# LPD-EPFL-ML/X-MAP

Measured on AMD Instinct MI355X. Metric: item_sim_pairs_per_s, higher is better.
Workload: dtype f64

## Files before the change

x-map_amd/csrc/tri_pairs.hip:

```cpp
#include <type_traits>

#include "tri.h"

namespace xmap {

constexpr uint32_t T_EMPTY = 0xFFFFFFFFu;

struct TriArgs {
    const long long *iptr;
    const RaterRec *rc;
    const int2 *ub;
    const double *u_avg; const double *nrm;
    int cap;
    const int *Q; const uint8_t *small; const int *uq_item; const int *uq_q; long long unit_lo, unit_hi;
    const int *hid; const int *hlist; const int *CH; const int *uc_item; const int *uc_c;
    const long long *uc_ptr; const int *C;
    double *hp_hi; double *hp_lo; int *hp_cnt; int *hp_mut;
    long long shard_cap;
    unsigned long long *shard_cur;
    unsigned long long *shard_occ;
    int *coo_i; int *coo_j; double *coo_sim; int *coo_mutu; int *coo_nij;
    double *coo_aux;
    int *rowcnt;
    int *mircnt;
    unsigned long long *counters;
    int heavy_mod, heavy_rem;
    int raw;
};

template <int METHOD>
__device__ __forceinline__ bool finish_pair(const TriArgs &A, int i, int j, int n, int m, double dot, double &simv) {
    const double np = A.nrm[i] * A.nrm[j];
    const double cs = (np != 0.0) ? 1.0 * dot / np : 0.0;
    const int mn = n < A.cap ? n : A.cap;
    simv = 1.0 * cs * (double)mn / (double)A.cap;
    return (simv != 0.0) && (m != 0);
}


template <typename Fin, typename Park, typename Get, typename Aux>
__device__ __forceinline__ void append_pairs(const TriArgs &A, int i, int s_begin, int n_slots, Fin fin, Park park, Get get,
                                             Aux aux) {
    const int lane = lane_id();
    const int shard = (blockIdx.x * (blockDim.x >> 6) + uniform((int)(threadIdx.x >> 6))) & (COO_SHARDS - 1);
    int kept = 0, occ = 0;
    for (int s0 = s_begin; s0 < n_slots; s0 += 64) {
        int j, n, m; double sv; bool o;
        bool keep = fin(s0 + lane, j, n, m, sv, o);
        park(s0 + lane, o, keep, sv);
        kept += __popcll(__ballot(keep));
        occ += __popcll(__ballot(o));
    }
    if (lane == 0 && occ) atomicAdd(&A.shard_occ[shard], (unsigned long long)occ);
    if (!kept) return;
    unsigned long long base = 0;
    if (lane == 0) {
        base = atomicAdd(&A.shard_cur[shard], (unsigned long long)kept);
        atomicAdd(&A.rowcnt[i], kept);
    }
    base = ((unsigned long long)(unsigned)rl32((int)(base >> 32), 0) << 32) | (unsigned)rl32((int)(base & 0xffffffffull), 0);
    if ((long long)(base + kept) > A.shard_cap) {
        if (lane == 0) atomicOr(&A.counters[3], 1ull);
        return;
    }
    base += (unsigned long long)shard * (unsigned long long)A.shard_cap;
    for (int s0 = s_begin; s0 < n_slots; s0 += 64) {
        int j, n, m; double sv;
        bool keep = get(s0 + lane, j, n, m, sv);
        unsigned long long km = __ballot(keep);
        if (keep) {
            long long p = (long long)base + __popcll(km & lanemask_lt());
            A.coo_i[p] = i; A.coo_j[p] = j;
            A.coo_sim[p] = sv; A.coo_mutu[p] = m; A.coo_nij[p] = n;
            if (A.coo_aux) A.coo_aux[p] = aux(s0 + lane);
        }
        base += __popcll(km);
    }
}

__global__ __launch_bounds__(256) void k_shard_sums(const unsigned long long *shards, unsigned long long *counters) {
    unsigned long long a = 0ull, b = 0ull;
    for (int s = threadIdx.x; s < COO_SHARDS; s += 256) { a += shards[s]; b += shards[COO_SHARDS + s]; }
    a = (unsigned long long)wave_sum_ll((long long)a);
    b = (unsigned long long)wave_sum_ll((long long)b);
    if (lane_id() == 0) { atomicAdd(&counters[4], a); atomicAdd(&counters[5], b); }
}



static_assert(std::is_standard_layout<TriArgs>::value, "KARG() addresses TriArgs fields by offsetof");
#define KARG(field) (*(decltype(TriArgs::field) const volatile __attribute__((address_space(4))) *)( \
    (const char __attribute__((address_space(4))) *)__builtin_amdgcn_kernarg_segment_ptr() + offsetof(TriArgs, field)))
template <int METHOD, int LOG_SLOTS, int NW, bool LS>
__global__ __launch_bounds__(64 * NW, (LOG_SLOTS == 7 && !LS) ? 8 : 1) void k_pair_tri(TriArgs A) {
    constexpr int SLOTS_ = 1 << LOG_SLOTS;
    constexpr bool ADJ = METHOD == XMAP_ADJUST_COSINE;
    using RT = typename std::conditional<LS, double, float>::type;
    using CM = typename std::conditional<NW == 16 || LS, unsigned long long, unsigned>::type;
    constexpr int MSH = (NW == 16 || LS) ? 32 : 16;
    constexpr CM NMASK = (CM)(((CM)1 << MSH) - 1);
    constexpr uint32_t LOCKBIT = 0x80000000u;
    __shared__ uint32_t key[SLOTS_];
    __shared__ CM cm[SLOTS_];
    __shared__ double dot[SLOTS_];
    __shared__ double dlo[ADJ ? SLOTS_ : 1];
    __shared__ unsigned short claim[ADJ && NW == 1 ? SLOTS_ : 1];
    __shared__ double s_ny[LS ? SLOTS_ : 1];
    __shared__ unsigned long long s_ls[LS ? SLOTS_ : 1];
    __shared__ int s_ovf;
    static_assert(!LS || ADJ, "the local-sensitivity pass keeps the similarity in dlo[]");

    const int lane = lane_id();
    const long long unit = A.unit_lo + blockIdx.x;
    if (unit >= A.unit_hi) return;
    const int i = uniform(A.uq_item[unit]);
    const int4 ud = ((const int4 *)A.uq_q)[unit];
    const int q = uniform(ud.x), p0 = uniform(ud.y), p1 = uniform(ud.z), Qi = uniform(ud.w);
    const int w = uniform((int)uniform((int)(threadIdx.x >> 6)));
    for (int s = threadIdx.x; s < SLOTS_; s += 64 * NW) {
        key[s] = T_EMPTY; cm[s] = (CM)0; dot[s] = 0.0;
        if (ADJ) dlo[s] = 0.0;
    }
    if (NW > 1) {
        if (threadIdx.x == 0) s_ovf = 0;
        __syncthreads();
    }
    const double nx = A.nrm[i];
    int ovf = 0;

    constexpr int RB = (NW == 1 || NW == 16) ? 64 : 16;
    constexpr int WU = 2;
    struct RawRec { int e0, pw, usr; RT r; };
    auto rater = [&](int p) {
        const int pc = (lane < RB && p < p1) ? p : p0;
        RawRec o;
        if (LS) {
            const RaterRecWide rr = ((const RaterRecWide *)A.rc)[pc];
            o.e0 = rr.e0; o.pw = rr.pos_ge; o.r = (RT)rr.rating; o.usr = 0;
        } else {
            const RaterRec rr = A.rc[pc];
            o.e0 = rr.e0; o.pw = rr.pos_ge; o.r = (RT)rr.rating; o.usr = rr.user;
        }
        return o;
    };
    auto entry = [&](int e, int &jw_, RT &rj_) {
        if (LS) { const UbWide v = ((const UbWide *)A.ub)[e]; jw_ = v.item_ge; rj_ = (RT)v.rating; }
        else { const int2 v = A.ub[e]; jw_ = v.x; rj_ = (RT)__int_as_float(v.y); }
    };
    auto walk = [&](auto &&body) {
        int base = p0 + RB * w;
        if (base >= p1) return;
        RawRec cur = rater(base + lane);
        for (; base < p1; base += RB * NW) {
            RawRec nxt = cur;
            if (base + RB * NW < p1) nxt = rater(base + RB * NW + lane);
            const bool ok = lane < RB && base + lane < p1;
            const int e0 = cur.e0, pw = cur.pw, usr = cur.usr;
            const RT r = cur.r;
            const int len = ok ? (pw & 0x7fffffff) : 0;
            int end = len;
#pragma unroll
            for (int d = 1; d < RB; d <<= 1) { const int v = __shfl_up(end, d, 64); if (lane >= d) end += v; }
            const int total = rl32(end, RB - 1);
            const int start = end - len;
            for (int f0 = 0; f0 < total; f0 += 64 * WU) {
                int jw[WU]; RT rj[WU]; bool act[WU]; double ri[WU], a[WU]; unsigned gei[WU];
                int tt[WU], ee[WU], uu[WU];
#pragma unroll
                for (int u = 0; u < WU; u++) {
                    const int f = f0 + u * 64 + lane;
                    act[u] = f < total;
// ... 165 lines not shown
        fj[t] = (int)kj;
        const CM c = cm[sl];
        fn[t] = (int)(c & NMASK); fm[t] = (int)(c >> MSH);
        fs[t] = dot[sl];
        fa[t] = (ADJ && k_raw) ? dlo[sl] : 0.0;
        fy[t] = 0.0;
        if (fo[t]) {
            if (!k_raw) fy[t] = k_nrm[kj];
        }
    }
    int kept = 0, occ = 0;
#pragma unroll
    for (int t = 0; t < NIT; t++) {
        bool keep = fo[t];
        if (keep && !k_raw) {
            const double np = nx * fy[t];
            const double cs = (np != 0.0) ? 1.0 * fs[t] / np : 0.0;
            const int mn = fn[t] < k_cap ? fn[t] : k_cap;
            fs[t] = 1.0 * cs * (double)mn / (double)k_cap;
            keep = (fs[t] != 0.0) && (fm[t] != 0);
        }
        fk[t] = keep;
        kept += __popcll(__ballot(keep));
        occ += __popcll(__ballot(fo[t]));
    }
    const int shard = (blockIdx.x * NW + w) & (COO_SHARDS - 1);
    if (lane == 0 && occ) atomicAdd(&k_shard_occ[shard], (unsigned long long)occ);
    if (!kept) return;
    unsigned long long cbase = 0;
    if (lane == 0) {
        cbase = atomicAdd(&k_shard_cur[shard], (unsigned long long)kept);
        atomicAdd(&k_rowcnt[i], kept);
    }
    cbase = ((unsigned long long)(unsigned)rl32((int)(cbase >> 32), 0) << 32) | (unsigned)rl32((int)(cbase & 0xffffffffull), 0);
    if ((long long)(cbase + kept) > k_shard_cap) {
        if (lane == 0) atomicOr(&k_counters[3], 1ull);
        return;
    }
    cbase += (unsigned long long)shard * (unsigned long long)k_shard_cap;
#pragma unroll
    for (int t = 0; t < NIT; t++) {
        const unsigned long long km = __ballot(fk[t]);
        if (fk[t]) {
            const long long pp = (long long)cbase + __popcll(km & lanemask_lt());
            const int j = fj[t];
            k_coo_i[pp] = i; k_coo_j[pp] = j;
            k_coo_sim[pp] = fs[t]; k_coo_mutu[pp] = fm[t]; k_coo_nij[pp] = fn[t];
            if (k_coo_aux) k_coo_aux[pp] = fa[t];
        }
        cbase += __popcll(km);
    }
}

constexpr int pack_lds(int log_slots, int g, int e) {
    return 8 * (g << log_slots) + 512 * e > (26 << log_slots) ? 8 * (g << log_slots) + 512 * e : (26 << log_slots);
}
constexpr int pack_waves(int lds) { return 160 * 1024 / lds / 4 > 8 ? 8 : 160 * 1024 / lds / 4; }
template <int METHOD, int LOG_SLOTS, int G, int PACK_E>
__global__ __launch_bounds__(64, pack_waves(pack_lds(LOG_SLOTS, G, PACK_E))) void k_pair_pack(TriArgs A) {
    constexpr int S = 1 << LOG_SLOTS, GS = G * S;
    constexpr int NIT = GS / 64;
    constexpr bool ADJ = METHOD == XMAP_ADJUST_COSINE;
    constexpr int CAP = 64 * PACK_E;
    static_assert(GS % 256 == 0 && GS <= 65536 && CAP <= 32768, "16-byte fills; (slot, rank) in one word");
    __shared__ __align__(16) unsigned char lds[pack_lds(LOG_SLOTS, G, PACK_E)];
    uint32_t *key = (uint32_t *)lds;
    uint32_t *cm = key + GS;
    double *terms = (double *)(cm + GS);
    uint32_t *key1 = (uint32_t *)lds;
    uint32_t *cm1 = key1 + S;
    double *dot1 = (double *)(cm1 + S);
    double *dlo1 = dot1 + S;
    unsigned short *claim1 = (unsigned short *)(dlo1 + S);

    const int lane = lane_id();
    const long long u0 = A.unit_lo + (long long)blockIdx.x * G;
    if (u0 >= A.unit_hi) return;
    const int nm = (A.unit_hi - u0 < G) ? (int)(A.unit_hi - u0) : G;
    const long long um = u0 + (lane < nm ? lane : 0);
    const int it_l = A.uq_item[um];
    const int4 ud = ((const int4 *)A.uq_q)[um];
    const int nr_l = lane < nm ? ud.z - ud.y : 0;
    int im[G], pm[G], ro[G + 1];
    ro[0] = 0;
#pragma unroll
    for (int m = 0; m < G; m++) {
        im[m] = rl32(it_l, m); pm[m] = rl32(ud.y, m);
        ro[m + 1] = ro[m] + rl32(nr_l, m);
    }
    const int R = ro[G];

    bool packed = R <= 64;
    int eoff = 0, usrf = 0, end = 0, total = 0;
    float r = 0.f;
    if (packed) {
        int p = pm[0] + lane;
#pragma unroll
        for (int m = 1; m < G; m++)
            if (lane >= ro[m]) p = pm[m] + (lane - ro[m]);
        const bool ok = lane < R;
        const RaterRec rr = A.rc[ok ? p : pm[0]];
        {
            const uint4 e4 = make_uint4(T_EMPTY, T_EMPTY, T_EMPTY, T_EMPTY), z4 = make_uint4(0u, 0u, 0u, 0u);
#pragma unroll
            for (int x = 0; x < GS / 256; x++) { ((uint4 *)key)[x * 64 + lane] = e4; ((uint4 *)cm)[x * 64 + lane] = z4; }
        }
        r = rr.rating;
        usrf = rr.user | (rr.pos_ge & (int)0x80000000);
        const int len = ok ? (rr.pos_ge & 0x7fffffff) : 0;
        end = len;
#pragma unroll
        for (int d = 1; d < 64; d <<= 1) { const int v = __shfl_up(end, d, 64); if (lane >= d) end += v; }
        total = rl32(end, 63);
        eoff = rr.e0 - (end - len);
        packed = total <= CAP;
    }
    if (!packed) {
        for (int m = 0; m < nm; m++) {
            const int i = rl32(it_l, m), p0 = rl32(ud.y, m), p1 = rl32(ud.z, m);
            int ovf = 0;
            __syncthreads();
            for (int s = lane; s < S; s += 64) { key1[s] = T_EMPTY; cm1[s] = 0u; dot1[s] = 0.0; dlo1[s] = 0.0; }
            __syncthreads();
            for (int base = p0; base < p1; base += 64) {
                const bool ok = base + lane < p1;
                const RaterRec rr = A.rc[ok ? base + lane : p0];
                const int len = ok ? (rr.pos_ge & 0x7fffffff) : 0;
                int en = len;
#pragma unroll
                for (int d = 1; d < 64; d <<= 1) { const int v = __shfl_up(en, d, 64); if (lane >= d) en += v; }
                const int tot = rl32(en, 63);
                const int st = en - len;
                for (int f0 = 0; f0 < tot; f0 += 64) {
                    const int f = f0 + lane;
                    bool act = f < tot;
                    int t = 0;
#pragma unroll
                    for (int step = 32; step >= 1; step >>= 1) { const int v = __shfl(en, t + step - 1, 64); if (v <= f) t += step; }
                    const int eb = __shfl(rr.e0, t, 64), sb = __shfl(st, t, 64), ut = __shfl(rr.user, t, 64);
                    const int pwt = __shfl(rr.pos_ge, t, 64);
                    const double ri = (double)__shfl(rr.rating, t, 64);
                    const int2 v = A.ub[act ? eb + (f - sb) : 0];
                    const double a = ADJ ? A.u_avg[act ? ut : 0] : 0.0;
                    const int j = v.x & 0x7fffffff;
                    const double rjd = (double)__int_as_float(v.y);
                    uint32_t h = 0;
                    if (act) {
                        h = ((uint32_t)j * 0x9E3779B1u) >> (32 - LOG_SLOTS);
                        int probes = 0;
                        for (;;) {
                            const uint32_t prev = atomicCAS(&key1[h], T_EMPTY, (uint32_t)j);
                            if (prev == T_EMPTY || prev == (uint32_t)j) break;
                            h = (h + 1) & (S - 1);
                            if (++probes >= S) { act = false; ovf = 1; break; }
                        }
                    }
                    if (act) atomicAdd(&cm1[h], 1u | (((((unsigned)v.x) >> 31) == (((unsigned)pwt) >> 31)) ? (1u << 16) : 0u));
                    const double tm = ADJ ? (ri - a) * (rjd - a) : (1.0 * ri) * rjd;
                    typedef __attribute__((address_space(3))) volatile double lds_vf64;
                    typedef __attribute__((address_space(3))) volatile unsigned short lds_vu16;
                    lds_vf64 *vhi = (lds_vf64 *)dot1, *vlo = (lds_vf64 *)dlo1;
                    lds_vu16 *vclaim = (lds_vu16 *)claim1;
                    bool pending = act;
                    while (__ballot(pending)) {
                        if (pending) vclaim[h] = (unsigned short)lane;
                        if (pending && vclaim[h] == (unsigned short)lane) {
                            double hi = vhi[h], lo = vlo[h];
                            dd_add(hi, lo, tm);
                            vhi[h] = hi; vlo[h] = lo;
                            pending = false;
// ... 296 lines not shown
            j = A.hlist[s]; n = (int)cnt[s]; m = (int)mut[s];
            return finish_pair<METHOD>(A, i, j, n, m, dot[s], sv);
        },
        [&](int s, bool o, bool keep, double sv) {
            if (o) { if (keep) dot[s] = sv; else cnt[s] = 0; }
        },
        [&](int s, int &j, int &n, int &m, double &sv) {
            if (cnt[s] == 0) return false;
            j = A.hlist[s]; n = (int)cnt[s]; m = (int)mut[s]; sv = dot[s];
            return true;
        },
        [&](int s) { return 0.0; });
}

}

using namespace xmap;

struct SideStreams { hipStream_t s[N_CLASSES + 1]; hipEvent_t fork, done[N_CLASSES + 1]; int dev; };
static SideStreams *side_streams() {
    static thread_local SideStreams *cur[64] = {nullptr};
    int dev = 0;
    if (hipGetDevice(&dev) != hipSuccess || dev < 0 || dev >= 64) { set_error("hipGetDevice failed"); return nullptr; }
    if (cur[dev]) return cur[dev];
    SideStreams *p = new SideStreams();
    p->dev = dev;
    bool ok = hipEventCreateWithFlags(&p->fork, hipEventDisableTiming) == hipSuccess;
    for (int c = 0; c <= N_CLASSES && ok; c++)
        ok = hipStreamCreateWithFlags(&p->s[c], hipStreamNonBlocking) == hipSuccess &&
             hipEventCreateWithFlags(&p->done[c], hipEventDisableTiming) == hipSuccess;
    if (!ok) { set_error("could not create the side streams"); delete p; return nullptr; }
    cur[dev] = p;
    return p;
}

namespace {

template <int METHOD, bool LS>
int launch_tri(int c, dim3 grid, hipStream_t st, const TriArgs &A) {
#define XM_TRI(LOG_SLOTS, NW) k_pair_tri<METHOD, LOG_SLOTS, NW, LS><<<grid, dim3(64 * NW), 0, st>>>(A)
    switch (c) {
    case 0: XM_TRI(10, 16); break;
    case 1: XM_TRI(10, 4); break;
    case 2: XM_TRI(9, 2); break;
    case 3: XM_TRI(8, 1); break;
    default: XM_TRI(7, 1); break;
    }
#undef XM_TRI
    XM_LAUNCH_CHECK();
    return XMAP_OK;
}

constexpr int PACK_G128 = 2, PACK_E128 = 3, PACK_G256 = 2, PACK_E256 = 6;
int pack_units(int c) { return c == 4 ? PACK_G128 : (c == 3 ? PACK_G256 : 0); }
template <int METHOD>
int launch_pack(int c, long long n_units, hipStream_t st, const TriArgs &A) {
    const int g = pack_units(c);
    const dim3 grid((unsigned)((n_units + g - 1) / g));
    if (c == 4) k_pair_pack<METHOD, 7, PACK_G128, PACK_E128><<<grid, dim3(64), 0, st>>>(A);
    else k_pair_pack<METHOD, 8, PACK_G256, PACK_E256><<<grid, dim3(64), 0, st>>>(A);
    XM_LAUNCH_CHECK();
    return XMAP_OK;
}

int launch_heavy(int method, hipStream_t st, const TriArgs &A, int n_units, int n_heavy) {
    const bool cos = method == XMAP_COSINE;
    if (n_units > 0) {
        (cos ? k_pair_heavy<XMAP_COSINE> : k_pair_heavy<XMAP_ADJUST_COSINE>)<<<dim3((unsigned)n_units), dim3(64 * HEAVY_WAVES), 0, st>>>(A);
        XM_LAUNCH_CHECK();
    }
    if (n_heavy > 0) {
        (cos ? k_heavy_merge<XMAP_COSINE> : k_heavy_merge<XMAP_ADJUST_COSINE>)<<<dim3((unsigned)n_heavy), dim3(256), 0, st>>>(A, n_heavy);
        XM_LAUNCH_CHECK();
    }
    return XMAP_OK;
}

}

extern "C" {

int xmap_sim2_pairs(void *stream, const xmap_ratings *R, int method, int cap, const double *u_avg, const double *norms, const void *rc,
                    const void *ub, const int32_t *Q, const uint8_t *small, const int32_t *uq_item, const int32_t *uq_q,
                    const int64_t *cls_ptr , int64_t unit_lo, int64_t unit_hi, const int32_t *hid, const int32_t *hlist,
                    const int32_t *ctl, const int32_t *C, const int64_t *uc_ptr, const int32_t *uc_item, const int32_t *uc_c,
                    int32_t n_heavy_units, int32_t n_heavy, int phases, double *hp_hi, double *hp_lo, int32_t *hp_cnt, int32_t *hp_mut,
                    int64_t coo_cap, int32_t *coo_i, int32_t *coo_j, double *coo_sim, int32_t *coo_mutu, int32_t *coo_nij,
                    double *coo_ls , int32_t *rowcnt, int64_t *d_shards , int64_t *d_counters ,
                    int32_t *mircnt ) {
    XM_SCOPE(stream);
    XM_ARG(R && u_avg && norms && rc && ub);
    XM_ARG(Q && small && uq_item && uq_q && cls_ptr && hid && hlist && ctl && C && uc_ptr && uc_item && uc_c);
    XM_ARG(coo_i && coo_j && coo_sim && coo_mutu && coo_nij && rowcnt && d_shards && d_counters);
    XM_ARG(coo_cap >= COO_SHARDS);
    XM_ARG(method == XMAP_COSINE || method == XMAP_ADJUST_COSINE || method == XMAP_COSINE_EXACT);
    XM_ARG(n_heavy_units == 0 || !(phases & (XMAP_PAIRS_HEAVY | XMAP_PAIRS_HEAVY_MERGE)) || (hp_hi && hp_lo && hp_cnt && hp_mut));
    hipStream_t st = (hipStream_t)stream;
    const bool exact_cos = method == XMAP_COSINE_EXACT;
    const double *nrm = norms + (method == XMAP_ADJUST_COSINE ? (size_t)R->n_items : 0);
    FillList F;
    if (exact_cos) {
        double *zero_avg = nullptr;
        const size_t ub = sizeof(double) * (size_t)(R->n_users > 0 ? R->n_users : 1);
        XM_HIP(xm_malloc_async((void **)&zero_avg, ub, st));
        F.add(zero_avg, ub);
        u_avg = zero_avg;
        method = XMAP_ADJUST_COSINE;
    }
    const bool raw = (phases & XMAP_PAIRS_RAW) != 0;
    XM_ARG(!coo_ls || ((raw || method == XMAP_ADJUST_COSINE) && n_heavy_units == 0));
    XM_ARG(!raw || (coo_ls && n_heavy_units == 0 && n_heavy == 0));
    const size_t In = (size_t)(R->n_items > 0 ? R->n_items : 1);
    const bool sums_cleared = (phases & XMAP_PAIRS_RESET) && (phases & XMAP_PAIRS_SHARD_SUMS);
    if (phases & XMAP_PAIRS_RESET) {
        F.add(d_counters, (sums_cleared ? 6 : 4) * sizeof(int64_t));
        F.add(d_shards, 2 * COO_SHARDS * sizeof(int64_t));
        if (!(phases & XMAP_PAIRS_NO_MARKS)) XM_HIP(hipMemsetAsync(coo_i, 0xff, sizeof(int32_t) * (size_t)coo_cap, st));
        F.add(rowcnt, sizeof(int32_t) * In);
        if (mircnt) F.add(mircnt, sizeof(int32_t) * In);
    }
    {
        int rc_fill = fill_multi(st, F);
        if (rc_fill) return rc_fill;
    }
    TriArgs A;
    memset(&A, 0, sizeof(A));
    A.iptr = (const long long *)R->item_ptr; A.rc = (const RaterRec *)rc; A.ub = (const int2 *)ub;
    A.u_avg = u_avg; A.nrm = nrm; A.cap = cap;
    A.Q = Q; A.small = small; A.uq_item = uq_item; A.uq_q = uq_q; A.unit_lo = unit_lo; A.unit_hi = unit_hi;
    A.hid = hid; A.hlist = hlist; A.CH = ctl; A.uc_item = uc_item; A.uc_c = uc_c;
    A.uc_ptr = (const long long *)uc_ptr; A.C = C;
    A.hp_hi = hp_hi; A.hp_lo = hp_lo; A.hp_cnt = hp_cnt; A.hp_mut = hp_mut;
    A.shard_cap = coo_cap / COO_SHARDS; A.shard_cur = (unsigned long long *)d_shards;
    A.shard_occ = (unsigned long long *)d_shards + COO_SHARDS;
    A.coo_i = coo_i; A.coo_j = coo_j; A.coo_sim = coo_sim; A.coo_mutu = coo_mutu; A.coo_nij = coo_nij; A.coo_aux = coo_ls; A.raw = raw ? 1 : 0;
    A.heavy_mod = XMAP_PAIRS_DEAL_MOD(phases); A.heavy_rem = XMAP_PAIRS_DEAL_REM(phases);
    if (A.heavy_mod < 1) A.heavy_mod = 1;
    A.rowcnt = rowcnt; A.mircnt = mircnt; A.counters = (unsigned long long *)d_counters;
    const int all_rows = XMAP_PAIRS_HEAVY | XMAP_PAIRS_LIGHT | XMAP_PAIRS_HEAVY_MERGE;
    const bool light = (phases & XMAP_PAIRS_LIGHT) && unit_hi > unit_lo;
    const bool heavy_aside = (phases & all_rows) == all_rows && n_heavy_units > 0 && unit_hi > unit_lo;
    hipStream_t hs = st;
    SideStreams *side = nullptr;
    if (light || heavy_aside) {
        side = side_streams();
        if (!side) return XMAP_ERR_HIP;
        XM_HIP(hipEventRecord(side->fork, st));
    }
    if (heavy_aside) {
        hs = side->s[N_CLASSES];
        XM_HIP(hipStreamWaitEvent(hs, side->fork, 0));
    }
    int rcode = launch_heavy(method, hs, A, (phases & XMAP_PAIRS_HEAVY) ? n_heavy_units : 0, heavy_aside ? n_heavy : 0);
    if (rcode) return rcode;
    if (heavy_aside) {
        XM_HIP(hipEventRecord(side->done[N_CLASSES], hs));
        XM_HIP(hipStreamWaitEvent(st, side->done[N_CLASSES], 0));
    }
    if (light) {
        const char *pk_env = getenv("XMAP_PAIR_PACKS");
        const bool packs = !raw && !coo_ls && !(pk_env && atoi(pk_env) == 0);
        for (int c = 0; c < N_CLASSES; c++) {
            const long long lo = unit_lo > cls_ptr[c] ? unit_lo : cls_ptr[c];
            const long long hi = unit_hi < cls_ptr[c + 1] ? unit_hi : cls_ptr[c + 1];
            if (hi <= lo) continue;
            A.unit_lo = lo; A.unit_hi = hi;
            const dim3 grid((unsigned)(hi - lo));
            hipStream_t cs = side->s[c];
            XM_HIP(hipStreamWaitEvent(cs, side->fork, 0));
            if (packs && pack_units(c))
                rcode = method == XMAP_COSINE ? launch_pack<XMAP_COSINE>(c, hi - lo, cs, A) : launch_pack<XMAP_ADJUST_COSINE>(c, hi - lo, cs, A);
            else if (coo_ls && !raw) rcode = launch_tri<XMAP_ADJUST_COSINE, true>(c, grid, cs, A);
            else if (method == XMAP_COSINE) rcode = launch_tri<XMAP_COSINE, false>(c, grid, cs, A);
            else rcode = launch_tri<XMAP_ADJUST_COSINE, false>(c, grid, cs, A);
            if (rcode) return rcode;
            XM_HIP(hipEventRecord(side->done[c], cs));
            XM_HIP(hipStreamWaitEvent(st, side->done[c], 0));
        }
        A.unit_lo = unit_lo; A.unit_hi = unit_hi;
    }
    if ((phases & XMAP_PAIRS_HEAVY_MERGE) && !heavy_aside && n_heavy_units > 0) {
        rcode = launch_heavy(method, st, A, 0, n_heavy);
        if (rcode) return rcode;
    }
    if (phases & XMAP_PAIRS_SHARD_SUMS) {
        if (!sums_cleared) XM_HIP(hipMemsetAsync(d_counters + 4, 0, 2 * sizeof(int64_t), st));
        k_shard_sums<<<dim3(1), dim3(256), 0, st>>>((const unsigned long long *)d_shards, (unsigned long long *)d_counters);
        XM_LAUNCH_CHECK();
    }
    if ((phases & XMAP_PAIRS_MIRCOUNT) && !raw && !mircnt && R->n_items > 0) {
        int *part = nullptr;
        XM_HIP(xm_malloc_async((void **)&part, sizeof(int) * (size_t)coo_cap, st));
        return mirror_counts(st, R->n_items, coo_cap / COO_SHARDS, COO_SHARDS, (const unsigned long long *)d_shards, coo_i, coo_j,
                             coo_ls != nullptr, part, rowcnt);
    }
    return XMAP_OK;
}

int xmap_sim3_counters_begin(void *stream, const int64_t *d_counters) {
    XM_ARG(d_counters);
    return host_wait_post((hipStream_t)stream, HW_PAIRS, d_counters, 6);
}
int xmap_sim3_counters_wait(int64_t *h_out) {
    XM_ARG(h_out);
    const int64_t *h = nullptr;
    int rcode = host_wait_take(HW_PAIRS, &h);
    if (rcode) return rcode;
    for (int c = 0; c < 6; c++) h_out[c] = h[c];
    return XMAP_OK;
}
}
```

x-map_amd/csrc/knn.hip:

```cpp
#include "paths.h"

namespace xmap {

__global__ __launch_bounds__(256) void k_bridge_flags(int I, const long long *row_ptr, const int *col,
                                                      const int *prefix_cls, uint8_t *bb) {
    int i = blockIdx.x * 4 + (threadIdx.x >> 6);
    if (i >= I) return;
    int lane = lane_id();
    long long lo = row_ptr[i], hi = row_ptr[i + 1];
    int pi = prefix_cls[i];
    int found = 0;
    for (long long b = lo; b < hi && !found; b += 64) {
        long long p = b + lane;
        int f = (p < hi) && (prefix_cls[col[p]] != pi);
        found = __ballot(f) != 0ull;
    }
    if (lane == 0) bb[i] = (uint8_t)found;
}

constexpr int K_THREADS = 256;
constexpr int K_CH = 2048;
constexpr int K_CH_SMALL = 512;
constexpr int K_WIN = 1024;

__device__ __forceinline__ bool before(unsigned long long ka, int ca, unsigned long long kb, int cb) {
    return (ka > kb) || (ka == kb && ca < cb);
}

__device__ __forceinline__ long long block_scan_ll(long long v, long long *total, long long *smem) {
    int lane = threadIdx.x & 63, w = threadIdx.x >> 6;
    long long inc = v;
#pragma unroll
    for (int d = 1; d < 64; d <<= 1) {
        long long o = __shfl_up(inc, d, 64);
        if (lane >= d) inc += o;
    }
    if (lane == 63) smem[w] = inc;
    __syncthreads();
    long long base = 0, tot = 0;
#pragma unroll
    for (int k = 0; k < K_THREADS / 64; k++) {
        long long s = smem[k];
        if (k < w) base += s;
        tot += s;
    }
    __syncthreads();
    *total = tot;
    return base + inc - v;
}

struct KnnArgs {
    int I, k, row_lo;
    const long long *row_ptr;
    const int *col;
    const double *sim;
    const int *mutu;
    const int *nij;
    const double *info;
    const double *frac;
    const uint8_t *bb;
    const int *suffix_cls;
    const uint32_t *contains_mask;
    uint8_t *cls;
    int *kcnt;
    int *kcol;
    double *kval;
};

template <int CH, int MODE>
__global__ __launch_bounds__(K_THREADS) void k_knn_classify(KnnArgs A) {
    __shared__ unsigned long long skey[CH];
    __shared__ int scol[CH];
    __shared__ int spos[CH];
    __shared__ long long sscan[4];
    __shared__ unsigned long long s_thrk[2];
    __shared__ int s_thrc[2], s_has[2], s_fill;

    const int i = blockIdx.x + A.row_lo;
    const int tid = threadIdx.x;
    const long long lo = A.row_ptr[i];
    const int n = (int)(A.row_ptr[i + 1] - lo);
    if ((MODE == 1 && n > CH) || (MODE == 2 && n <= K_CH_SMALL)) return;
    const int k = A.k;
    auto zero_tail = [&](int nA, int nB) {
        for (int e = tid; e < 2 * k; e += K_THREADS) {
            const int l = e >= k, r = e - l * k;
            if (r < (l ? nB : nA)) continue;
            const size_t o = ((size_t)i * 2 + l) * k + r;
            A.kcol[o] = 0; A.kval[o * 3] = 0.0; A.kval[o * 3 + 1] = 0.0; A.kval[o * 3 + 2] = 0.0;
        }
    };
    if (n == 0) {
        if (tid == 0) {
            A.cls[i] = 0;
            A.kcnt[(size_t)i * 2] = 0;
            A.kcnt[(size_t)i * 2 + 1] = 0;
        }
        zero_tail(0, 0);
        return;
    }
    const bool isbb = A.bb[i] != 0;
    const int sc = A.suffix_cls[i];
    if (tid < 2) s_has[tid] = 0;
    int nc = 0, consumed = 0;
    for (;;) {
        int total;
        if (consumed == 0 || CH - nc < K_WIN) {
            const int take = (CH - nc) < (n - consumed) ? (CH - nc) : (n - consumed);
            for (int t = tid; t < take; t += K_THREADS) {
                int p = consumed + t;
                double s = A.sim[lo + p];
                skey[nc + t] = (unsigned long long)__double_as_longlong(fabs(s));
                scol[nc + t] = A.col[lo + p];
                spos[nc + t] = p;
            }
            total = nc + take;
            consumed += take;
        } else {
            if (tid == 0) s_fill = nc;
            __syncthreads();
            for (;;) {
                const int f = s_fill;
                __syncthreads();
                if (consumed >= n || CH - f < K_WIN) break;
#pragma unroll
                for (int u = 0; u < K_WIN / K_THREADS; u++) {
                    const int p = consumed + tid + K_THREADS * u;
                    if (p < n) {
                        const unsigned long long key = (unsigned long long)__double_as_longlong(fabs(A.sim[lo + p]));
                        const int c = A.col[lo + p];
                        bool pa, pb;
                        if (isbb) {
                            bool has = (A.contains_mask[c] >> sc) & 1u;
                            pa = !has; pb = has;
                        } else {
                            pa = A.bb[c] != 0; pb = true;
                        }
                        const bool keep = (pa && (!s_has[0] || before(key, c, s_thrk[0], s_thrc[0]))) ||
                                          (pb && (!s_has[1] || before(key, c, s_thrk[1], s_thrc[1])));
                        if (keep) {
                            const int o = atomicAdd(&s_fill, 1);
                            skey[o] = key; scol[o] = c; spos[o] = p;
                        }
                    }
                }
                consumed = (consumed + K_WIN) < n ? (consumed + K_WIN) : n;
                __syncthreads();
            }
            total = s_fill;
        }
        int N = 2;
        while (N < total) N <<= 1;
        for (int t = total + tid; t < N; t += K_THREADS) {
            skey[t] = 0ull;
            scol[t] = 0x7fffffff;
            spos[t] = -1;
        }
        __syncthreads();
        if (N <= 128) {
            if (tid < 64) {
                for (int k2 = 2; k2 <= N; k2 <<= 1) {
                    for (int j = k2 >> 1; j > 0; j >>= 1) {
                        const int t = tid;
                        if (t < (N >> 1)) {
                            int a = 2 * t - (t & (j - 1));
                            int b = a + j;
                            bool up = (a & k2) == 0;
                            unsigned long long ka = skey[a], kb = skey[b];
                            int ca = scol[a], cb = scol[b];
                            bool sw = up ? before(kb, cb, ka, ca) : before(ka, ca, kb, cb);
                            if (sw) {
                                skey[a] = kb; skey[b] = ka;
                                scol[a] = cb; scol[b] = ca;
                                int pa = spos[a], pb = spos[b];
                                spos[a] = pb; spos[b] = pa;
                            }
                        }
                        __builtin_amdgcn_fence(__ATOMIC_RELEASE, "wavefront");
                        __builtin_amdgcn_wave_barrier();
                        __builtin_amdgcn_fence(__ATOMIC_ACQUIRE, "wavefront");
                    }
                }
            }
            __syncthreads();
        } else
        for (int k2 = 2; k2 <= N; k2 <<= 1) {
            for (int j = k2 >> 1; j > 0; j >>= 1) {
                for (int t = tid; t < (N >> 1); t += K_THREADS) {
                    int a = 2 * t - (t & (j - 1));
                    int b = a + j;
                    bool up = (a & k2) == 0;
                    unsigned long long ka = skey[a], kb = skey[b];
                    int ca = scol[a], cb = scol[b];
                    bool sw = up ? before(kb, cb, ka, ca) : before(ka, ca, kb, cb);
                    if (sw) {
                        skey[a] = kb; skey[b] = ka;
                        scol[a] = cb; scol[b] = ca;
                        int pa = spos[a], pb = spos[b];
                        spos[a] = pb; spos[b] = pa;
// ... 35 lines not shown
                if ((pa && rA < k) || (pb && rB < k)) {
                    double sv = A.sim[p];
                    double mu = (double)A.mutu[p];
                    double fr = A.frac ? A.frac[p]
                                       : 1.0 * mu / (A.info[(size_t)i * 4 + 3] + A.info[(size_t)c * 4 + 3] - (double)A.nij[p]);
                    if (pa && rA < k) {
                        size_t o = ((size_t)i * 2 + 0) * k + rA;
                        A.kcol[o] = c; A.kval[o * 3] = sv; A.kval[o * 3 + 1] = mu; A.kval[o * 3 + 2] = fr;
                    }
                    if (pb && rB < k) {
                        size_t o = ((size_t)i * 2 + 1) * k + rB;
                        A.kcol[o] = c; A.kval[o * 3] = sv; A.kval[o * 3 + 1] = mu; A.kval[o * 3 + 2] = fr;
                    }
                }
                rA += pa; rB += pb;
            }
            if (tid == 0) {
                int nA = totA < k ? totA : k, nB = totB < k ? totB : k;
                uint8_t c = isbb ? 1 : (nA > 0 ? 2 : 0);
                A.cls[i] = c;
                A.kcnt[(size_t)i * 2] = c ? nA : 0;
                A.kcnt[(size_t)i * 2 + 1] = c ? nB : 0;
            }
            zero_tail(totA < k ? totA : k, totB < k ? totB : k);
            return;
        }
        unsigned long long rk[CH / K_THREADS];
        int rc[CH / K_THREADS], rp[CH / K_THREADS];
        int nk = 0;
        for (int t = s0; t < s0 + per && t < total; t++) {
            int c = scol[t];
            bool pa, pb;
            if (isbb) {
                bool has = (A.contains_mask[c] >> sc) & 1u;
                pa = !has; pb = has;
            } else {
                pa = A.bb[c] != 0; pb = true;
            }
            if ((pa && rA < k) || (pb && rB < k)) { rk[nk] = skey[t]; rc[nk] = c; rp[nk] = spos[t]; nk++; }
            if (pa && rA == k - 1) { s_thrk[0] = skey[t]; s_thrc[0] = c; s_has[0] = 1; }
            if (pb && rB == k - 1) { s_thrk[1] = skey[t]; s_thrc[1] = c; s_has[1] = 1; }
            rA += pa; rB += pb;
        }
        long long tk;
        long long ek = block_scan_ll((long long)nk, &tk, sscan);
        for (int q = 0; q < nk; q++) {
            skey[ek + q] = rk[q]; scol[ek + q] = rc[q]; spos[ek + q] = rp[q];
        }
        nc = (int)tk;
        __syncthreads();
    }
}

__global__ __launch_bounds__(256) void k_knn_thresholds(int I, int k, const int *kcnt, const int *kcol, const double *kval, KnnThr *thr) {
    const long long t = (long long)blockIdx.x * blockDim.x + threadIdx.x;
    if (t >= 2ll * I) return;
    KnnThr th;
    th.cnt = kcnt[t]; th.col = 0; th.la = 0.0;
    if (th.cnt > 0) {
        const size_t o = (size_t)t * k + (th.cnt - 1);
        th.la = fabs(kval[o * 3]); th.col = kcol[o];
    }
    thr[t] = th;
}

}

using namespace xmap;

extern "C" {

int xmap_bridge_flags(void *stream, const xmap_sim *S, const int32_t *prefix_cls, uint8_t *bb) {
    XM_ARG(S && prefix_cls && bb);
    if (S->n_items == 0) return XMAP_OK;
    k_bridge_flags<<<dim3((unsigned)((S->n_items + 3) / 4)), dim3(256), 0, (hipStream_t)stream>>>(
        S->n_items, (const long long *)S->row_ptr, S->col, prefix_cls, bb);
    XM_LAUNCH_CHECK();
    return XMAP_OK;
}

int xmap_knn_classify(void *stream, const xmap_sim *S, int top_k, const uint8_t *bb, const int32_t *suffix_cls,
                      const uint32_t *contains_mask, uint8_t *cls, int32_t *kcnt, int32_t *kcol, double *kval,
                      int32_t row_lo, int32_t row_hi) {
    XM_ARG(S && bb && suffix_cls && contains_mask && cls && kcnt && kcol && kval);
    XM_ARG(top_k >= 1 && 2 * top_k <= K_CH / 2);
    XM_ARG(row_lo >= 0 && row_lo <= row_hi && row_hi <= S->n_items);
    if (row_hi == row_lo) return XMAP_OK;
    KnnArgs A;
    A.I = S->n_items; A.k = top_k; A.row_lo = row_lo;
    A.row_ptr = (const long long *)S->row_ptr; A.col = S->col; A.sim = S->sim; A.mutu = S->mutu; A.nij = S->nij;
    A.info = S->info; A.frac = S->frac; A.bb = bb; A.suffix_cls = suffix_cls; A.contains_mask = contains_mask;
    A.cls = cls; A.kcnt = kcnt; A.kcol = kcol; A.kval = kval;
    if (2 * top_k <= K_CH_SMALL / 2) {
        k_knn_classify<K_CH_SMALL, 1><<<dim3((unsigned)(row_hi - row_lo)), dim3(K_THREADS), 0, (hipStream_t)stream>>>(A);
        XM_LAUNCH_CHECK();
        k_knn_classify<K_CH, 2><<<dim3((unsigned)(row_hi - row_lo)), dim3(K_THREADS), 0, (hipStream_t)stream>>>(A);
    } else {
        k_knn_classify<K_CH, 0><<<dim3((unsigned)(row_hi - row_lo)), dim3(K_THREADS), 0, (hipStream_t)stream>>>(A);
    }
    XM_LAUNCH_CHECK();
    return XMAP_OK;
}

int xmap_knn_thresholds(void *stream, int32_t n_items, int top_k, const int32_t *kcnt, const int32_t *kcol, const double *kval,
                        void *thr) {
    XM_ARG(kcnt && kcol && kval && thr);
    if (n_items == 0) return XMAP_OK;
    k_knn_thresholds<<<dim3((unsigned)((2ll * n_items + 255) / 256)), dim3(256), 0, (hipStream_t)stream>>>(
        n_items, top_k, kcnt, kcol, kval, (KnnThr *)thr);
    XM_LAUNCH_CHECK();
    return XMAP_OK;
}

}
```

Measured before the change: 28.64 billion.

## Route small 512-slot units through a packed kernel, leave the rest to tri

```diff
diff --git a/x-map_amd/csrc/tri_pairs.hip b/x-map_amd/csrc/tri_pairs.hip
--- a/x-map_amd/csrc/tri_pairs.hip
+++ b/x-map_amd/csrc/tri_pairs.hip
@@ -26,6 +26,7 @@
     unsigned long long *counters;
     int heavy_mod, heavy_rem;
     int raw;
+    int pack_cap;
 };
 
 template <int METHOD>
@@ -117,6 +118,17 @@
     const int4 ud = ((const int4 *)A.uq_q)[unit];
     const int q = uniform(ud.x), p0 = uniform(ud.y), p1 = uniform(ud.z), Qi = uniform(ud.w);
     const int w = uniform((int)uniform((int)(threadIdx.x >> 6)));
+    if (LOG_SLOTS == 9 && !LS) {
+        const int pcap = KARG(pack_cap);
+        if (pcap > 0 && p1 - p0 <= 64) {
+            const bool ok = lane < p1 - p0;
+            const RaterRec rr = A.rc[ok ? p0 + lane : p0];
+            int tot = ok ? (rr.pos_ge & 0x7fffffff) : 0;
+#pragma unroll
+            for (int d = 32; d >= 1; d >>= 1) tot += __shfl_xor(tot, d, 64);
+            if (rl32(tot, 0) <= pcap) return;
+        }
+    }
     for (int s = threadIdx.x; s < SLOTS_; s += 64 * NW) {
         key[s] = T_EMPTY; cm[s] = (CM)0; dot[s] = 0.0;
         if (ADJ) dlo[s] = 0.0;
@@ -388,18 +400,19 @@
     }
 }
 
-constexpr int pack_lds(int log_slots, int g, int e) {
-    return 8 * (g << log_slots) + 512 * e > (26 << log_slots) ? 8 * (g << log_slots) + 512 * e : (26 << log_slots);
+constexpr int pack_lds(int log_slots, int g, int e, bool fb) {
+    return (!fb || 8 * (g << log_slots) + 512 * e > (26 << log_slots)) ? 8 * (g << log_slots) + 512 * e : (26 << log_slots);
 }
 constexpr int pack_waves(int lds) { return 160 * 1024 / lds / 4 > 8 ? 8 : 160 * 1024 / lds / 4; }
-template <int METHOD, int LOG_SLOTS, int G, int PACK_E>
-__global__ __launch_bounds__(64, pack_waves(pack_lds(LOG_SLOTS, G, PACK_E))) void k_pair_pack(TriArgs A) {
+template <int METHOD, int LOG_SLOTS, int G, int PACK_E, bool FB>
+__global__ __launch_bounds__(64, pack_waves(pack_lds(LOG_SLOTS, G, PACK_E, FB))) void k_pair_pack(TriArgs A) {
     constexpr int S = 1 << LOG_SLOTS, GS = G * S;
     constexpr int NIT = GS / 64;
     constexpr bool ADJ = METHOD == XMAP_ADJUST_COSINE;
     constexpr int CAP = 64 * PACK_E;
     static_assert(GS % 256 == 0 && GS <= 65536 && CAP <= 32768, "16-byte fills; (slot, rank) in one word");
-    __shared__ __align__(16) unsigned char lds[pack_lds(LOG_SLOTS, G, PACK_E)];
+    static_assert(FB || G == 1, "k_pair_tri tells the packed kernel's units apart one by one");
+    __shared__ __align__(16) unsigned char lds[pack_lds(LOG_SLOTS, G, PACK_E, FB)];
     uint32_t *key = (uint32_t *)lds;
     uint32_t *cm = key + GS;
     double *terms = (double *)(cm + GS);
@@ -451,7 +464,8 @@
         eoff = rr.e0 - (end - len);
         packed = total <= CAP;
     }
-    if (!packed) {
+    if (!FB && !packed) return;
+    if (FB && !packed) {
         for (int m = 0; m < nm; m++) {
             const int i = rl32(it_l, m), p0 = rl32(ud.y, m), p1 = rl32(ud.z, m);
             int ovf = 0;
@@ -854,15 +868,24 @@
 }
 
 constexpr int PACK_G128 = 2, PACK_E128 = 3, PACK_G256 = 2, PACK_E256 = 6;
-int pack_units(int c) { return c == 4 ? PACK_G128 : (c == 3 ? PACK_G256 : 0); }
+constexpr int PACK_G512 = 1, PACK_E512 = 6;
+int pack_units(int c) { return c == 4 ? PACK_G128 : (c == 3 ? PACK_G256 : (c == 2 ? PACK_G512 : 0)); }
 template <int METHOD>
 int launch_pack(int c, long long n_units, hipStream_t st, const TriArgs &A) {
     const int g = pack_units(c);
     const dim3 grid((unsigned)((n_units + g - 1) / g));
-    if (c == 4) k_pair_pack<METHOD, 7, PACK_G128, PACK_E128><<<grid, dim3(64), 0, st>>>(A);
-    else k_pair_pack<METHOD, 8, PACK_G256, PACK_E256><<<grid, dim3(64), 0, st>>>(A);
+    if (c == 4) k_pair_pack<METHOD, 7, PACK_G128, PACK_E128, true><<<grid, dim3(64), 0, st>>>(A);
+    else if (c == 3) k_pair_pack<METHOD, 8, PACK_G256, PACK_E256, true><<<grid, dim3(64), 0, st>>>(A);
+    else k_pair_pack<METHOD, 9, PACK_G512, PACK_E512, false><<<grid, dim3(64), 0, st>>>(A);
     XM_LAUNCH_CHECK();
     return XMAP_OK;
+}
+
+template <int METHOD>
+int launch_long512(long long n_units, hipStream_t st, const TriArgs &A) {
+    TriArgs T = A;
+    T.pack_cap = 64 * PACK_E512;
+    return launch_tri<METHOD, false>(2, dim3((unsigned)n_units), st, T);
 }
 
 int launch_heavy(int method, hipStream_t st, const TriArgs &A, int n_units, int n_heavy) {
@@ -962,6 +985,8 @@
     if (light) {
         const char *pk_env = getenv("XMAP_PAIR_PACKS");
         const bool packs = !raw && !coo_ls && !(pk_env && atoi(pk_env) == 0);
+        const char *big_env = getenv("XMAP_PAIR_BIG");
+        const bool big = packs && !(big_env && atoi(big_env) == 0);
         for (int c = 0; c < N_CLASSES; c++) {
             const long long lo = unit_lo > cls_ptr[c] ? unit_lo : cls_ptr[c];
             const long long hi = unit_hi < cls_ptr[c + 1] ? unit_hi : cls_ptr[c + 1];
@@ -970,7 +995,11 @@
             const dim3 grid((unsigned)(hi - lo));
             hipStream_t cs = side->s[c];
             XM_HIP(hipStreamWaitEvent(cs, side->fork, 0));
-            if (packs && pack_units(c))
+            if (packs && c == 2 && big) {
+                rcode = method == XMAP_COSINE ? launch_long512<XMAP_COSINE>(hi - lo, cs, A) : launch_long512<XMAP_ADJUST_COSINE>(hi - lo, cs, A);
+                if (rcode) return rcode;
+            }
+            if (packs && pack_units(c) && (c != 2 || big))
                 rcode = method == XMAP_COSINE ? launch_pack<XMAP_COSINE>(c, hi - lo, cs, A) : launch_pack<XMAP_ADJUST_COSINE>(c, hi - lo, cs, A);
             else if (coo_ls && !raw) rcode = launch_tri<XMAP_ADJUST_COSINE, true>(c, grid, cs, A);
             else if (method == XMAP_COSINE) rcode = launch_tri<XMAP_COSINE, false>(c, grid, cs, A);
```

Measured after the change: 28.96 billion (median of 6 runs). No clear change (+1.1%).

## Bin KNN rows by length and process short rows with one wave each

Applied to the files above, without the earlier changes.

```diff
diff --git a/x-map_amd/csrc/knn.hip b/x-map_amd/csrc/knn.hip
--- a/x-map_amd/csrc/knn.hip
+++ b/x-map_amd/csrc/knn.hip
@@ -20,8 +20,10 @@
 
 constexpr int K_THREADS = 256;
 constexpr int K_CH = 2048;
-constexpr int K_CH_SMALL = 512;
-constexpr int K_WIN = 1024;
+constexpr int K_CH_HALF = 1024;
+constexpr int K_HALF_BLOCKS = 5;
+constexpr int K_CAP_A = 256, K_CAP_B = 512, K_VLONG = 8192;
+constexpr int K_NCLS = 4;
 
 __device__ __forceinline__ bool before(unsigned long long ka, int ca, unsigned long long kb, int cb) {
     return (ka > kb) || (ka == kb && ca < cb);
@@ -50,7 +52,13 @@
 }
 
 struct KnnArgs {
-    int I, k, row_lo;
+    int I, k;
+    int first;
+    const int *list;
+    const unsigned *count;
+    const int *list0;
+    const unsigned *count0;
+    unsigned *ticket;
     const long long *row_ptr;
     const int *col;
     const double *sim;
@@ -67,20 +75,217 @@
     double *kval;
 };
 
-template <int CH, int MODE>
-__global__ __launch_bounds__(K_THREADS) void k_knn_classify(KnnArgs A) {
+constexpr int K_LIST_R = 16;
+__global__ __launch_bounds__(256) void k_knn_list_rows(int row_lo, int row_hi, const long long *row_ptr, int cap_a, int cap_b,
+                                                       int cap_v, int *lists, long long stride, unsigned *count) {
+    const int lane = lane_id();
+    const long long first = (long long)row_lo + ((long long)blockIdx.x * 4 + (threadIdx.x >> 6)) * (64 * K_LIST_R) + lane;
+    int c[K_LIST_R];
+    unsigned base[K_NCLS];
+#pragma unroll
+    for (int q = 0; q < K_NCLS; q++) base[q] = 0;
+#pragma unroll
+    for (int u = 0; u < K_LIST_R; u++) {
+        const long long i = first + 64 * u;
+        c[u] = -1;
+        if (i < row_hi) {
+            const long long n = row_ptr[i + 1] - row_ptr[i];
+            c[u] = n <= cap_a ? 0 : (n <= cap_b ? 1 : (n <= cap_v ? 2 : 3));
+        }
+#pragma unroll
+        for (int q = 0; q < K_NCLS; q++) base[q] += (unsigned)__popcll(__ballot(c[u] == q));
+    }
+#pragma unroll
+    for (int q = 0; q < K_NCLS; q++) {
+        unsigned b = 0;
+        if (lane == 0 && base[q] > 0) b = atomicAdd(&count[q], base[q]);
+        base[q] = (unsigned)__shfl((int)b, 0, 64);
+    }
+#pragma unroll
+    for (int u = 0; u < K_LIST_R; u++) {
+#pragma unroll
+        for (int q = 0; q < K_NCLS; q++) {
+            const unsigned long long m = __ballot(c[u] == q);
+            if (c[u] == q) lists[(long long)q * stride + base[q] + __popcll(m & lanemask_lt())] = (int)(first + 64 * u);
+            base[q] += (unsigned)__popcll(m);
+        }
+    }
+}
+
+template <int CAP>
+__global__ __launch_bounds__(K_THREADS, (160 * 1024 / (CAP * 16 * (K_THREADS / 64)) > 8 ? 8 : 160 * 1024 / (CAP * 16 * (K_THREADS / 64))))
+void k_knn_rows_wave(KnnArgs A) {
+    constexpr int U = CAP / 64 > 0 ? CAP / 64 : 1;
+    constexpr int LCAP = CAP < 64 ? 64 : CAP;
+    __shared__ ulonglong2 sent_[K_THREADS / 64][LCAP];
+    const int lane = lane_id(), w = uniform(threadIdx.x >> 6);
+    ulonglong2 *sent = sent_[w];
+    const int k = A.k;
+    const unsigned count = *A.count;
+    auto wave_fence = [] {
+        __builtin_amdgcn_fence(__ATOMIC_RELEASE, "wavefront");
+        __builtin_amdgcn_wave_barrier();
+        __builtin_amdgcn_fence(__ATOMIC_ACQUIRE, "wavefront");
+    };
+    for (unsigned idx = blockIdx.x * (K_THREADS / 64) + w; idx < count; idx += gridDim.x * (K_THREADS / 64)) {
+        const int i = A.list[idx];
+        const long long lo = A.row_ptr[i];
+        const int n = (int)(A.row_ptr[i + 1] - lo);
+        auto zero_tail = [&](int nA, int nB) {
+            for (int e = lane; e < 2 * k; e += 64) {
+                const int l = e >= k, r = e - l * k;
+                if (r < (l ? nB : nA)) continue;
+                const size_t o = ((size_t)i * 2 + l) * k + r;
+                A.kcol[o] = 0; A.kval[o * 3] = 0.0; A.kval[o * 3 + 1] = 0.0; A.kval[o * 3 + 2] = 0.0;
+            }
+        };
+        if (n == 0) {
+            if (lane == 0) {
+                A.cls[i] = 0;
+                A.kcnt[(size_t)i * 2] = 0;
+                A.kcnt[(size_t)i * 2 + 1] = 0;
+            }
+            zero_tail(0, 0);
+            continue;
+        }
+        const bool isbb = A.bb[i] != 0;
+        const int sc = A.suffix_cls[i];
+        int N = 2;
+        while (N < n) N <<= 1;
+        {
+            double ls[U];
+            int lc[U];
+#pragma unroll
+            for (int u = 0; u < U; u++) {
+                const int t = lane + 64 * u, tc = t < n ? t : n - 1;
+                ls[u] = A.sim[lo + tc]; lc[u] = A.col[lo + tc];
+            }
+#pragma unroll
+            for (int u = 0; u < U; u++) {
+                const int t = lane + 64 * u;
+                ulonglong2 e;
+                e.x = t < n ? (unsigned long long)__double_as_longlong(fabs(ls[u])) : 0ull;
+                e.y = t < n ? ((unsigned long long)(unsigned)lc[u] << 32) | (unsigned)t : 0x7fffffffffffffffull;
+                if (t < N) sent[t] = e;
+            }
+        }
+        wave_fence();
+        auto cex = [&](int t, int j, int k2) {
+            const int a = 2 * t - (t & (j - 1));
+            const int b = a + j;
+            const ulonglong2 ea = sent[a], eb = sent[b];
+            const bool a_first = (ea.x > eb.x) || (ea.x == eb.x && ea.y < eb.y);
+            if (a_first != ((a & k2) == 0)) { sent[a] = eb; sent[b] = ea; }
+        };
+        const int half = N >> 1;
+        if (half <= 64) {
+            for (int k2 = 2; k2 <= N; k2 <<= 1) {
+                for (int j = k2 >> 1; j > 0; j >>= 1) {
+                    if (lane < half) cex(lane, j, k2);
+                    wave_fence();
+                }
+            }
+        } else {
+            for (int k2 = 2; k2 <= N; k2 <<= 1) {
+                for (int j = k2 >> 1; j > 0; j >>= 1) {
+                    for (int t0 = 0; t0 < half; t0 += 64) cex(t0 + lane, j, k2);
+                    wave_fence();
+                }
+            }
+        }
+        const int per = N > 64 ? (N >> 6) : 1;
+        const int s0 = lane * per;
+        unsigned pm = 0;
+        int cA = 0, cB = 0;
+        {
+            unsigned wd[U];
+            if (isbb) {
+#pragma unroll
+                for (int u = 0; u < U; u++) {
+                    const bool ok = u < per && s0 + u < n;
+                    wd[u] = A.contains_mask[(int)(sent[ok ? s0 + u : 0].y >> 32)];
+                }
+            } else {
+#pragma unroll
+                for (int u = 0; u < U; u++) {
+                    const bool ok = u < per && s0 + u < n;
+                    wd[u] = A.bb[(int)(sent[ok ? s0 + u : 0].y >> 32)];
+                }
+            }
+#pragma unroll
+            for (int u = 0; u < U; u++) {
+                if (u < per && s0 + u < n) {
+                    bool pa, pb;
+                    if (isbb) {
+                        const bool has = (wd[u] >> sc) & 1u;
+                        pa = !has; pb = has;
+                    } else {
+                        pa = wd[u] != 0; pb = true;
+                    }
+                    pm |= ((unsigned)pa << u) | ((unsigned)pb << (16 + u));
+                    cA += pa; cB += pb;
+                }
+            }
+        }
+        const int v = cA | (cB << 16);
+        int inc = v;
+#pragma unroll
+        for (int d = 1; d < 64; d <<= 1) {
+            int o = __shfl_up(inc, d, 64);
+            if (lane >= d) inc += o;
+        }
+        const int tot = __shfl(inc, 63, 64);
+        int rA = (inc - v) & 0xffff, rB = (inc - v) >> 16;
+        const int totA = tot & 0xffff, totB = tot >> 16;
+#pragma unroll 1
+        for (int u = 0; u < per; u++) {
+            if (s0 + u < n) {
+                const bool pa = (pm >> u) & 1u, pb = (pm >> (16 + u)) & 1u;
+                if ((pa && rA < k) || (pb && rB < k)) {
+                    const unsigned long long y = sent[s0 + u].y;
+                    const int c = (int)(y >> 32);
+                    const long long p = lo + (int)(unsigned)y;
+                    double sv = A.sim[p];
+                    double mu = (double)A.mutu[p];
+                    double fr = A.frac ? A.frac[p]
+                                       : 1.0 * mu / (A.info[(size_t)i * 4 + 3] + A.info[(size_t)c * 4 + 3] - (double)A.nij[p]);
+                    if (pa && rA < k) {
+                        size_t o = ((size_t)i * 2 + 0) * k + rA;
+                        A.kcol[o] = c; A.kval[o * 3] = sv; A.kval[o * 3 + 1] = mu; A.kval[o * 3 + 2] = fr;
+                    }
+                    if (pb && rB < k) {
+                        size_t o = ((size_t)i * 2 + 1) * k + rB;
+                        A.kcol[o] = c; A.kval[o * 3] = sv; A.kval[o * 3 + 1] = mu; A.kval[o * 3 + 2] = fr;
+                    }
+                }
+                rA += pa; rB += pb;
+            }
+        }
+        const int nA = totA < k ? totA : k, nB = totB < k ? totB : k;
+        if (lane == 0) {
+            uint8_t c = isbb ? 1 : (nA > 0 ? 2 : 0);
+            A.cls[i] = c;
+            A.kcnt[(size_t)i * 2] = c ? nA : 0;
+            A.kcnt[(size_t)i * 2 + 1] = c ? nB : 0;
+        }
+        zero_tail(nA, nB);
+        wave_fence();
+    }
+}
+
+template <int CH>
+__device__ __forceinline__ void knn_row_block(const KnnArgs &A, const int i) {
     __shared__ unsigned long long skey[CH];
     __shared__ int scol[CH];
     __shared__ int spos[CH];
     __shared__ long long sscan[4];
     __shared__ unsigned long long s_thrk[2];
     __shared__ int s_thrc[2], s_has[2], s_fill;
-
-    const int i = blockIdx.x + A.row_lo;
+    constexpr int WIN = CH / 2;
+
     const int tid = threadIdx.x;
     const long long lo = A.row_ptr[i];
     const int n = (int)(A.row_ptr[i + 1] - lo);
-    if ((MODE == 1 && n > CH) || (MODE == 2 && n <= K_CH_SMALL)) return;
     const int k = A.k;
     auto zero_tail = [&](int nA, int nB) {
         for (int e = tid; e < 2 * k; e += K_THREADS) {
@@ -105,8 +310,9 @@
     int nc = 0, consumed = 0;
     for (;;) {
         int total;
-        if (consumed == 0 || CH - nc < K_WIN) {
-            const int take = (CH - nc) < (n - consumed) ? (CH - nc) : (n - consumed);
+        if (consumed == 0 || CH - nc < WIN) {
+            const int room = consumed == 0 ? A.first : CH - nc;
+            const int take = room < (n - consumed) ? room : (n - consumed);
             for (int t = tid; t < take; t += K_THREADS) {
                 int p = consumed + t;
                 double s = A.sim[lo + p];
@@ -119,32 +325,52 @@
         } else {
             if (tid == 0) s_fill = nc;
             __syncthreads();
+            const bool hasA = s_has[0] != 0, hasB = s_has[1] != 0;
+            const unsigned long long thrkA = s_thrk[0], thrkB = s_thrk[1];
+            const int thrcA = s_thrc[0], thrcB = s_thrc[1];
+            constexpr int WU = WIN / K_THREADS;
+            double ws[WU];
+            int wc[WU];
+            auto request = [&](unsigned from) {
+#pragma unroll
+                for (int u = 0; u < WU; u++) {
+                    const unsigned p = from + tid + K_THREADS * u;
+                    if (p < (unsigned)n) { ws[u] = A.sim[lo + p]; wc[u] = A.col[lo + p]; }
+                }
+            };
+            request((unsigned)consumed);
             for (;;) {
                 const int f = s_fill;
                 __syncthreads();
-                if (consumed >= n || CH - f < K_WIN) break;
-#pragma unroll
-                for (int u = 0; u < K_WIN / K_THREADS; u++) {
+                if (consumed >= n || CH - f < WIN) break;
+                double cs[WU];
+                int cc[WU];
+#pragma unroll
+                for (int u = 0; u < WU; u++) { cs[u] = ws[u]; cc[u] = wc[u]; }
+                request((unsigned)consumed + WIN);
+#pragma unroll
+                for (int u = 0; u < WU; u++) {
                     const int p = consumed + tid + K_THREADS * u;
                     if (p < n) {
-                        const unsigned long long key = (unsigned long long)__double_as_longlong(fabs(A.sim[lo + p]));
-                        const int c = A.col[lo + p];
-                        bool pa, pb;
-                        if (isbb) {
-                            bool has = (A.contains_mask[c] >> sc) & 1u;
-                            pa = !has; pb = has;
-                        } else {
-                            pa = A.bb[c] != 0; pb = true;
+                        const unsigned long long key = (unsigned long long)__double_as_longlong(fabs(cs[u]));
+                        const int c = cc[u];
+                        const bool ta = !hasA || before(key, c, thrkA, thrcA), tb = !hasB || before(key, c, thrkB, thrcB);
+                        if (ta || tb) {
+                            bool pa, pb;
+                            if (isbb) {
+                                bool has = (A.contains_mask[c] >> sc) & 1u;
+                                pa = !has; pb = has;
+                            } else {
+                                pa = A.bb[c] != 0; pb = true;
+                            }
+                            if ((pa && ta) || (pb && tb)) {
+                                const int o = atomicAdd(&s_fill, 1);
+                                skey[o] = key; scol[o] = c; spos[o] = p;
+                            }
                         }
-                        const bool keep = (pa && (!s_has[0] || before(key, c, s_thrk[0], s_thrc[0]))) ||
-                                          (pb && (!s_has[1] || before(key, c, s_thrk[1], s_thrc[1])));
-                        if (keep) {
-                            const int o = atomicAdd(&s_fill, 1);
-                            skey[o] = key; scol[o] = c; spos[o] = p;
-                        }
-                    }
-                }
-                consumed = (consumed + K_WIN) < n ? (consumed + K_WIN) : n;
+                    }
+                }
+                consumed = (consumed + WIN) < n ? (consumed + WIN) : n;
                 __syncthreads();
             }
             total = s_fill;
@@ -286,6 +512,20 @@
     }
 }
 
+template <int CH>
+__global__ __launch_bounds__(K_THREADS, CH <= K_CH_HALF ? K_HALF_BLOCKS : 4) void k_knn_classify(KnnArgs A) {
+    __shared__ unsigned s_ticket;
+    const unsigned count0 = *A.count0, count = *A.count;
+    for (;;) {
+        if (threadIdx.x == 0) s_ticket = atomicAdd(A.ticket, 1u);
+        __syncthreads();
+        const unsigned t = s_ticket;
+        if (t >= count0 + count) break;
+        knn_row_block<CH>(A, t < count0 ? A.list0[t] : A.list[t - count0]);
+        __syncthreads();
+    }
+}
+
 __global__ __launch_bounds__(256) void k_knn_thresholds(int I, int k, const int *kcnt, const int *kcol, const double *kval, KnnThr *thr) {
     const long long t = (long long)blockIdx.x * blockDim.x + threadIdx.x;
     if (t >= 2ll * I) return;
@@ -316,21 +556,50 @@
 int xmap_knn_classify(void *stream, const xmap_sim *S, int top_k, const uint8_t *bb, const int32_t *suffix_cls,
                       const uint32_t *contains_mask, uint8_t *cls, int32_t *kcnt, int32_t *kcol, double *kval,
                       int32_t row_lo, int32_t row_hi) {
+    XM_SCOPE(stream);
     XM_ARG(S && bb && suffix_cls && contains_mask && cls && kcnt && kcol && kval);
     XM_ARG(top_k >= 1 && 2 * top_k <= K_CH / 2);
     XM_ARG(row_lo >= 0 && row_lo <= row_hi && row_hi <= S->n_items);
     if (row_hi == row_lo) return XMAP_OK;
+    hipStream_t st = (hipStream_t)stream;
+    const long long n_rows = (long long)row_hi - row_lo;
+    int dev = 0, cus = 0;
+    XM_HIP(hipGetDevice(&dev));
+    XM_HIP(hipDeviceGetAttribute(&cus, hipDeviceAttributeMultiprocessorCount, dev));
+    if (cus < 1) cus = 1;
+    int *lists = nullptr;
+    unsigned *count = nullptr;
+    XM_HIP(xm_malloc_async((void **)&lists, sizeof(int) * (size_t)K_NCLS * (size_t)n_rows, st));
+    XM_HIP(xm_malloc_async((void **)&count, sizeof(unsigned) * (K_NCLS + 1), st));
+    XM_HIP(hipMemsetAsync(count, 0, sizeof(unsigned) * (K_NCLS + 1), st));
+    k_knn_list_rows<<<dim3(blocks_for(n_rows, 256 * K_LIST_R)), dim3(256), 0, st>>>(
+        row_lo, row_hi, (const long long *)S->row_ptr, K_CAP_A, K_CAP_B, K_VLONG, lists, n_rows, count);
+    XM_LAUNCH_CHECK();
     KnnArgs A;
-    A.I = S->n_items; A.k = top_k; A.row_lo = row_lo;
+    A.I = S->n_items; A.k = top_k;
+    A.first = K_CAP_B;
+    while (A.first < 8 * top_k && A.first < K_CH) A.first <<= 1;
     A.row_ptr = (const long long *)S->row_ptr; A.col = S->col; A.sim = S->sim; A.mutu = S->mutu; A.nij = S->nij;
     A.info = S->info; A.frac = S->frac; A.bb = bb; A.suffix_cls = suffix_cls; A.contains_mask = contains_mask;
     A.cls = cls; A.kcnt = kcnt; A.kcol = kcol; A.kval = kval;
-    if (2 * top_k <= K_CH_SMALL / 2) {
-        k_knn_classify<K_CH_SMALL, 1><<<dim3((unsigned)(row_hi - row_lo)), dim3(K_THREADS), 0, (hipStream_t)stream>>>(A);
-        XM_LAUNCH_CHECK();
-        k_knn_classify<K_CH, 2><<<dim3((unsigned)(row_hi - row_lo)), dim3(K_THREADS), 0, (hipStream_t)stream>>>(A);
+    A.list0 = nullptr; A.count0 = nullptr; A.ticket = nullptr;
+    auto grid = [&](int per_cu, int rows_per_block) {
+        const long long full = (long long)cus * per_cu, need = (n_rows + rows_per_block - 1) / rows_per_block;
+        return dim3((unsigned)(need < full ? need : full));
+    };
+    constexpr int WPB = K_THREADS / 64;
+    A.list = lists; A.count = count;
+    k_knn_rows_wave<K_CAP_A><<<grid(8, WPB), dim3(K_THREADS), 0, st>>>(A);
+    XM_LAUNCH_CHECK();
+    A.list = lists + n_rows; A.count = count + 1;
+    k_knn_rows_wave<K_CAP_B><<<grid(5, WPB), dim3(K_THREADS), 0, st>>>(A);
+    XM_LAUNCH_CHECK();
+    A.list = lists + 2 * n_rows; A.count = count + 2;
+    A.list0 = lists + 3 * n_rows; A.count0 = count + 3; A.ticket = count + K_NCLS;
+    if (2 * top_k <= K_CH_HALF / 4) {
+        k_knn_classify<K_CH_HALF><<<grid(K_HALF_BLOCKS, 1), dim3(K_THREADS), 0, st>>>(A);
     } else {
-        k_knn_classify<K_CH, 0><<<dim3((unsigned)(row_hi - row_lo)), dim3(K_THREADS), 0, (hipStream_t)stream>>>(A);
+        k_knn_classify<K_CH><<<grid(4, 1), dim3(K_THREADS), 0, st>>>(A);
     }
     XM_LAUNCH_CHECK();
     return XMAP_OK;
```

New measurement: 28.63 billion before, 28.65 billion after, median of 3. No clear change (+0.1%).
